# dgkuester/iqwaveform

Measured on NVIDIA B200. Metric: complex IQ GS/s for persistence_spectrum, higher is better.
Workload: dtype f32

## Files before the change

### include/iqw_b200.h

```cpp
#ifndef IQW_B200_H
#define IQW_B200_H

#include <stddef.h>
#include <stdint.h>

#ifdef __cplusplus
extern "C" {
#endif

#define IQW_ABI_VERSION 8

typedef enum iqw_status {
    IQW_OK = 0,
    IQW_ERR_INVALID = -1,
    IQW_ERR_UNSUPPORTED = -2,
    IQW_ERR_CUDA = -3,
    IQW_ERR_WORKSPACE = -4
} iqw_status;

typedef enum iqw_stft_mode {
    IQW_STFT_COMPLEX = 0,
    IQW_STFT_POWER = 1,
    IQW_STFT_DB = 2
} iqw_stft_mode;
// ... 72 lines not shown
                       const float* d_window, int32_t nfft, int64_t hop, int64_t n_frames,
                       int32_t bin_lo, int32_t bin_hi, void* d_out, int64_t out_channel_stride,
                       void* stream);


int iqw_edge_counts_f32(const float* d_a, int64_t n_rows, int64_t n_cols, const double* d_edges,
                        int32_t n_edges, int32_t side_right, int64_t* d_counts, void* stream);

size_t iqw_bracket_collect_workspace_bytes(int64_t n_rows, int64_t n_cols);
int iqw_bracket_collect_f32(const float* d_p, int64_t n_rows, int64_t n_cols, int32_t n_sel,
                            const uint32_t* d_lo, const uint32_t* d_hi, int32_t* d_below,
                            void* d_workspace, size_t workspace_bytes, void* stream);
int iqw_candidate_count_f32(const void* d_workspace, int64_t n_rows, int64_t n_cols, int32_t n_sel,
                            const uint32_t* d_lo, const uint32_t* d_hi, int32_t level,
                            int32_t* d_counts, void* stream);
int iqw_radix_count_f32(const float* d_p, int64_t n_rows, int64_t n_cols, int32_t n_sel,
                        const uint32_t* d_lo, const uint32_t* d_hi, int32_t level,
                        int32_t* d_counts, int32_t* d_below, void* stream);
int iqw_radix_descend(const int32_t* d_counts, int32_t n_sel, int64_t n_cols, int32_t level,
                      int64_t* d_rank, uint32_t* d_prefix, uint32_t* d_lo, uint32_t* d_hi,
                      void* stream);
int iqw_order_stats_finish_f32(const uint32_t* d_keys, int32_t n_sel, const int64_t* sel_rank,
                               int64_t n_rows_total, int64_t n_cols, const iqw_stat* stats,
                               int32_t n_stats, int32_t to_dB, float eps, float* d_out, void* stream);

int iqw_debug_set_stft_scratch_cap(size_t bytes);

int iqw_debug_set_sample_min_rows(int64_t rows);

int iqw_debug_set_stft_variant(int variant);

int iqw_debug_set_sample_margin(double sigmas, int extra_ranks);

int iqw_debug_time_stats_counters(const void* d_workspace, int64_t n_cols, uint32_t* host_out16);

int iqw_profile_enable(int level);
int iqw_profile_reset(void);
int iqw_profile_report(char* buf, size_t capacity);

#ifdef __cplusplus
}
#endif
#endif
```

### iqwaveform_b200/_lib.py

```python
from __future__ import annotations

import ctypes
import os

import torch

_HERE = os.path.dirname(os.path.abspath(__file__))
LIB_PATH = os.environ.get('IQW_B200_LIB') or os.path.join(_HERE, 'libiqw_b200.so')

ABI_VERSION = 8

IQW_OK = 0
IQW_ERR_INVALID = -1
IQW_ERR_UNSUPPORTED = -2
IQW_ERR_CUDA = -3
IQW_ERR_WORKSPACE = -4

STFT_COMPLEX, STFT_POWER, STFT_DB = 0, 1, 2
STAT_QUANTILE, STAT_MEAN, STAT_MAX, STAT_MIN, STAT_MEDIAN, STAT_ORDER = 0, 1, 2, 3, 4, 5
EW_POWTODB, EW_DBTOPOW, EW_ENVTOPOW, EW_ENVTODB = 0, 1, 2, 3

MAX_RANKS_PER_CALL = 8


# ... 17 lines not shown
                                    _i32, _i32, _vp, _i64, _vp, _sz, _vp]),
    'iqw_stft_bluestein_c64': (ctypes.c_int, [_vp, _i64, _i64, _i64, _vp, _vp, _vp, _i32, _i32, _i64, _i64, _i32, _f32,
                                              _i32, _i32, _vp, _i64, _vp]),
    'iqw_bluestein_pre_c64': (ctypes.c_int, [_vp, _i64, _vp, _i32, _i32, _i64, _vp, _vp]),
    'iqw_bluestein_mul_c64': (ctypes.c_int, [_vp, _vp, _i32, _i64, _vp]),
    'iqw_bluestein_post_c64': (ctypes.c_int, [_vp, _vp, _i32, _i64, _i32, _f32, _i32, _i32, _vp, _vp]),
    'iqw_stft_reduce_workspace_bytes': (_sz, [_i32]),
    'iqw_stft_reduce_c64': (ctypes.c_int, [_vp, _i64, _i64, _i64, _vp, _i32, _i64, _i64, _i32, _f32, _i32, _i32,
                                           ctypes.POINTER(iqw_stat), _i32, _vp, _vp, _sz, _vp]),
    'iqw_time_stats_workspace_bytes': (_sz, [_i64, _i64, _i64, _i32]),
    'iqw_time_stats_f32': (ctypes.c_int, [_vp, _i64, _i64, _i64, _i64, ctypes.POINTER(iqw_stat),
                                          _i32, _i32, _f32, _vp, _vp, _sz, _vp]),
    'iqw_bin_power_workspace_bytes': (_sz, [_i64, _i64, _i64]),
    'iqw_bin_power_c64': (ctypes.c_int, [_vp, _i64, _i64, _i64, _i64, _vp, _vp, _vp, _vp, _sz, _vp]),
    'iqw_envtopow_transposed_c64': (ctypes.c_int, [_vp, _i64, _i64, _i64, _i64, _vp, _vp]),
    'iqw_elementwise_f32': (ctypes.c_int, [_i32, _vp, _vp, _i64, _i32, _f32, _vp]),
    'iqw_elementwise_c64': (ctypes.c_int, [_i32, _vp, _vp, _i64, _f32, _vp]),
    'iqw_transpose_c64': (ctypes.c_int, [_vp, _i64, _i64, _i64, _vp, _vp]),
    'iqw_istft_c64': (ctypes.c_int, [_vp, _i64, _i64, _i64, _i32, _i64, _i32, _i32, _i32, _vp, _f32, _vp, _i64, _vp]),
    'iqw_ifft_c64': (ctypes.c_int, [_vp, _i64, _i32, _vp, _vp]),
    'iqw_ola_filter_c64': (ctypes.c_int, [_vp, _i64, _i64, _i64, _vp, _i32, _i64, _i64, _i32, _i32, _vp, _i64, _vp]),
    'iqw_edge_counts_f32': (ctypes.c_int, [_vp, _i64, _i64, _vp, _i32, _i32, _vp, _vp]),
    'iqw_bracket_collect_workspace_bytes': (_sz, [_i64, _i64]),
    'iqw_bracket_collect_f32': (ctypes.c_int, [_vp, _i64, _i64, _i32, _vp, _vp, _vp, _vp, _sz, _vp]),
    'iqw_candidate_count_f32': (ctypes.c_int, [_vp, _i64, _i64, _i32, _vp, _vp, _i32, _vp, _vp]),
    'iqw_radix_count_f32': (ctypes.c_int, [_vp, _i64, _i64, _i32, _vp, _vp, _i32, _vp, _vp, _vp]),
    'iqw_radix_descend': (ctypes.c_int, [_vp, _i32, _i64, _i32, _vp, _vp, _vp, _vp, _vp]),
    'iqw_order_stats_finish_f32': (ctypes.c_int, [_vp, _i32, ctypes.POINTER(_i64), _i64, _i64,
                                                  ctypes.POINTER(iqw_stat), _i32, _i32, _f32, _vp, _vp]),
    'iqw_debug_set_stft_scratch_cap': (ctypes.c_int, [_sz]),
    'iqw_debug_set_stft_variant': (ctypes.c_int, [ctypes.c_int]),
    'iqw_debug_set_sample_min_rows': (ctypes.c_int, [_i64]),
    'iqw_debug_set_sample_margin': (ctypes.c_int, [ctypes.c_double, ctypes.c_int]),
    'iqw_debug_time_stats_counters': (ctypes.c_int, [_vp, _i64, ctypes.POINTER(ctypes.c_uint32)]),
    'iqw_profile_enable': (ctypes.c_int, [ctypes.c_int]),
    'iqw_profile_reset': (ctypes.c_int, []),
    'iqw_profile_report': (ctypes.c_int, [ctypes.c_char_p, _sz]),
}


def _load() -> ctypes.CDLL:
    if not os.path.exists(LIB_PATH):
        raise ImportError(
            f'{LIB_PATH} is missing: build it with `python -c "import __graft_entry__ as g; '
            f'g.build()"` or `make -C iqwaveform_b200/csrc`.  iqwaveform_b200 has no CPU fallback.'
        )
    lib = ctypes.CDLL(LIB_PATH)
    for name, (restype, argtypes) in SIGNATURES.items():
        try:
            fn = getattr(lib, name)
        except AttributeError as exc:
            raise ImportError(f'{LIB_PATH} does not export {name}') from exc
        fn.restype = restype
        fn.argtypes = argtypes
    got = lib.iqw_abi_version()
    if got != ABI_VERSION:
        raise ImportError(f'{LIB_PATH}: ABI version {got}, python layer expects {ABI_VERSION}')
    return lib


lib = _load()


class IQWError(RuntimeError):
    pass

# ... 26 lines not shown
```

### iqwaveform_b200/csrc/iqw_stats.cu

```cuda
#include <cmath>
#include <atomic>
#include <cooperative_groups.h>
#include "iqw_common.cuh"

namespace iqw {

constexpr int kMaxRanks = 8;
constexpr int kMaxStats = 32;
constexpr int kNB0 = 256;
constexpr int kNSub = 32;
constexpr int kCap = 2048;
constexpr int kRefineLevels = 7;
constexpr int kBX = 128;
#ifndef IQW_UNROLL
#define IQW_UNROLL 8
#endif
constexpr int kUnroll = IQW_UNROLL;
constexpr long long kSampleMinRows = 16384;
constexpr int kSampleRows = 8192;
#ifndef IQW_SAMPLE_COLS
#define IQW_SAMPLE_COLS 2
#endif
constexpr int kSampleCols = IQW_SAMPLE_COLS;
constexpr int kMaxGroups = 8;
constexpr int kSelBins = 2048;
constexpr int kSubBins = 256;
#ifndef IQW_SEL_BUF
#define IQW_SEL_BUF 2048
#endif
#ifndef IQW_SEL_THREADS
#define IQW_SEL_THREADS 512
#endif
// ... 361 lines not shown
        }
        cum = next;
    }
    iv_store(L, w, col);
}

__device__ void scan_refine_body(long long col, long long cols, const RankPlan& rp, const Work& w) {
    if (col >= cols) return;
    IvList O, L;
    iv_load(O, w, col);
    bool any = false;
    for (uint32_t v = 0; v < O.n; ++v) any |= O.status[v] == IV_REFINE;
    if (!any) return;
    L.n = 0;
    for (uint32_t v = 0; v < O.n; ++v) {
        if (O.status[v] != IV_REFINE) {
            const uint32_t i = L.n++;
            L.klo[i] = O.klo[v]; L.khi[i] = O.khi[v]; L.shift[i] = O.shift[v]; L.below[i] = O.below[v];
            L.status[i] = O.status[v]; L.first[i] = O.first[v]; L.nr[i] = O.nr[v]; L.cnt[i] = O.cnt[v];
            continue;
        }
        atomicSub(w.pending, 1u);
        uint32_t cum = O.below[v], i = O.first[v];
        split_by_subbuckets(L, O, v, w.hist1 + (col * kMaxRanks + v) * kNSub, rp, i, cum, w, col);
    }
    iv_store(L, w, col);
}

__global__ void scan_refine_kernel(long long cols, RankPlan rp, Work w) {
    if (*w.pending == 0) return;
    scan_refine_body((long long)blockIdx.x * blockDim.x + threadIdx.x, cols, rp, w);
}

__global__ void scan_brackets_kernel(long long cols, long long rows, RankPlan rp, int n_groups,
                                     Work w) {
    const long long col = (long long)blockIdx.x * blockDim.x + threadIdx.x;
    if (col >= cols) return;
    IvList L;
    L.n = 0;
    uint32_t i = 0;
    const uint32_t nrk = (uint32_t)rp.n_ranks;
    const uint32_t ovf = w.t_ovf[col];
    bool first_live = true;
    for (int g = 0; g < n_groups && i < nrk; ++g) {
        const uint32_t lo = w.bk_lo[col * kMaxGroups + g], hi = w.bk_hi[col * kMaxGroups + g];
        if (lo > hi) continue;
        const uint32_t below = w.t_below[col * kMaxGroups + g];
        unsigned long long next_lo = 0x100000000ull;
        uint32_t next_below = (uint32_t)rows;
        for (int h = g + 1; h < n_groups; ++h) {
            const uint32_t l2 = w.bk_lo[col * kMaxGroups + h];
            if (l2 <= w.bk_hi[col * kMaxGroups + h]) { next_lo = l2; next_below = w.t_below[col * kMaxGroups + h]; break; }
        }
        if (first_live && rp.rank[i] < below) {
            const uint32_t first = i;
            while (i < nrk && rp.rank[i] < below) ++i;
            atomicAdd(w.pending + 2, i - first);
            iv_append(L, w, col, 0u, (unsigned long long)lo, 0u, below, first, i - first, false, 0u);
        }
        first_live = false;
        if (i < nrk && rp.rank[i] < next_below) {
            const uint32_t first = i;
            while (i < nrk && rp.rank[i] < next_below) ++i;
            const uint32_t region = next_below - below;
            if (ovf) {
                atomicAdd(w.pending + 3, 1u);
                iv_append(L, w, col, lo, next_lo - lo, below, region, first, i - first, false, 0u);
            } else {
                const uint32_t v = L.n++;
                L.klo[v] = lo; L.khi[v] = hi; L.below[v] = below; L.cnt[v] = region;
// ... 91 lines not shown
refine_kernel(const float* __restrict__ p, long long cols, RowMap rm, long long rows_per_split,
              Work w) {
    if (*w.pending == 0) return;
    extern __shared__ uint16_t hist[];
    refine_body<M>(blockIdx.x, blockIdx.y, gridDim.x, p, cols, rm, rows_per_split, w, hist);
}

#include "bracket_visit.inc"

template <bool RAW, int M>
__device__ __forceinline__ void bracket_visit_generic(uint32_t v, float (&nge)[M], float (&nin)[M],
                                                      uint32_t& slot, const uint32_t (&lo)[M],
                                                      const uint32_t (&hi)[M], uint32_t base) {
    bool inside = false;
#pragma unroll
    for (int g = 0; g < M; ++g) {
        const bool ge = RAW ? (int32_t)v >= (int32_t)lo[g] : v >= lo[g];
        const bool in = ge && (RAW ? (int32_t)v <= (int32_t)hi[g] : v <= hi[g]);
        nge[g] += ge ? 1.f : 0.f;
        nin[g] += in ? 1.f : 0.f;
        inside |= in;
    }
    if (inside) {
        asm volatile("st.shared.u32 [%0], %1;" :: "r"(base + 4 * slot), "r"(v) : "memory");
        slot += 1;
    }
}

constexpr int kLine = 32;
constexpr int kStage = kLine + kUnroll;
constexpr int kStagePitch = kStage + 1;

template <int M, int NAMED , bool RAW>
__device__ __forceinline__ void bracket_pass_body(const float* __restrict__ p, long long cols, long long col,
                                                  bool live_col, long long i0, long long i1, float eps,
                                                  const BracketPlan& bp, const Work& w, uint32_t* stage) {
    uint32_t lo[M], hi[M];
    float n_ge[M], n_in[M];
#pragma unroll
    for (int g = 0; g < M; ++g) {
        lo[g] = (live_col ? w.bk_lo[col * kMaxGroups + g] : 0xFFFFFFFFu) ^ (RAW ? 0x80000000u : 0u);
        hi[g] = (live_col ? w.bk_hi[col * kMaxGroups + g] : 0u) ^ (RAW ? 0x80000000u : 0u);
        n_ge[g] = 0.f; n_in[g] = 0.f;
    }
    const uint32_t cap = bp.cap_sum;
    const int lane = threadIdx.x & 31;
    uint32_t* my_stage = stage + threadIdx.x * kStagePitch;
    const uint32_t* warp_stage = stage + (threadIdx.x - lane) * kStagePitch;
    const uint32_t stage_addr = (uint32_t)__cvta_generic_to_shared(my_stage);
    uint32_t slot = 0;
    uint32_t n_lines = 0;
    uint32_t* warp_list = w.lists + ((long long)blockIdx.y * cols + (long long)blockIdx.x * kBX +
                                     (threadIdx.x - lane)) * (long long)cap;
    Named<(NAMED & 1) != 0, (NAMED & 2) != 0, (NAMED & 4) != 0> named;

    auto drain = [&](bool ready) {
        unsigned m = __ballot_sync(0xFFFFFFFFu, ready);
        __syncwarp();
        while (m) {
            const int src = __ffs(m) - 1;
            m &= m - 1;
            const uint32_t start = __shfl_sync(0xFFFFFFFFu, n_lines, src) * kLine;
            if (start + kLine <= cap)
                warp_list[(uint32_t)src * cap + start + lane] = warp_stage[src * kStagePitch + lane];
        }
        __syncwarp();
        if (ready) {
            const uint32_t left = slot - kLine;
            uint32_t t[kUnroll];
#pragma unroll
            for (int j = 0; j < kUnroll; ++j) t[j] = my_stage[kLine + j];
#pragma unroll
            for (int j = 0; j < kUnroll; ++j)
                if ((uint32_t)j < left) my_stage[j] = t[j];
            slot -= kLine;
            ++n_lines;
        }
    };
    auto visit = [&](float f) {
        const uint32_t bits = __float_as_uint(f);
        if (NAMED) named.add(f, float_to_key(f), eps);
        const uint32_t v = RAW ? bits : float_to_key(f);
        if constexpr (M <= 4) bracket_visit<RAW>(v, n_ge, n_in, slot, lo, hi, stage_addr);
        else bracket_visit_generic<RAW, M>(v, n_ge, n_in, slot, lo, hi, stage_addr);
    };
// ... 113 lines not shown
        for (int u = 0; u < kBpUnroll; ++u) visit(f[u]);
        drain(kChunk);
    };
    if (i + kBpUnroll <= i1) load_block(fa);
#pragma unroll 1
    while (i + kBpUnroll <= i1) {
        if (i + 2 * kBpUnroll <= i1) load_block(fb);
        visit_block(fa);
        i += kBpUnroll;
        if (i + kBpUnroll > i1) break;
        if (i + 2 * kBpUnroll <= i1) load_block(fa);
        visit_block(fb);
        i += kBpUnroll;
    }
#pragma unroll 1
    for (; i < i1; ++i, src += cols) {
        visit(__ldcs(src));
    }
    drain(kChunk);
    const uint32_t n_list = p4 >> 2;
    drain(1u);
    if (!live_col) return;

#pragma unroll
    for (int g = 0; g < M; ++g)
        if (g < bp.n_groups && wd[g] != 0u && nlt[g]) atomicAdd(w.t_below + col * kMaxGroups + g, nlt[g]);
    w.s_cnt[(long long)blockIdx.y * cols + col] = min(n_list, cap);
    if (n_list > cap) atomicOr(w.t_ovf + col, 1u);
    named.flush(w, col);
}

template <int M, int NAMED>
__global__ void __launch_bounds__(kBX)
bracket_pass_kernel(const float* __restrict__ p, long long cols, long long rows,
                    long long rows_per_split, float eps, BracketPlan bp, Work w) {
    static_assert(kRing <= kStagePitch, "the staging area serves both bodies");
    __shared__ __align__(128) uint32_t stage[kBX * kStagePitch];
    long long col = (long long)blockIdx.x * kBX + threadIdx.x;
    const bool live_col = col < cols;
    if (!live_col) col = cols - 1;
    const long long i0 = (long long)blockIdx.y * rows_per_split;
    const long long i1 = min(rows, i0 + rows_per_split);
    if (w.pending[8] == 0) {
        if constexpr (M <= 4) bracket_pass_body_diff<M, NAMED>(p, cols, col, live_col, i0, i1, eps, bp, w, stage);
        else bracket_pass_body<M, NAMED, true>(p, cols, col, live_col, i0, i1, eps, bp, w, stage);
    } else {
        bracket_pass_body<M, NAMED, false>(p, cols, col, live_col, i0, i1, eps, bp, w, stage);
    }
}

template <int M>
__device__ __forceinline__ void collect_body(unsigned bx, unsigned by, unsigned gdx, const float* __restrict__ p,
                                             long long cols, RowMap rm, long long rows_per_split, const Work& w) {
    const long long col_tiles = (cols + kBX - 1) / kBX;
    const long long i0 = (long long)by * rows_per_split;
    const long long i1 = min(rm.n, i0 + rows_per_split);
    for (long long tile = bx; tile < col_tiles; tile += gdx) {
        const long long col = tile * kBX + threadIdx.x;
        int active = 0;
        IvRegs<M> iv;
        iv.load(w, col, col < cols, IV_COLLECT, active);
        if (!__syncthreads_or(active)) continue;
        if (!active) continue;
        auto visit = [&](float f) {
            const uint32_t k = float_to_key(f);
            uint32_t kl, kh, sh;
            const int v = iv.find(k, kl, kh, sh);
            if (v >= 0 && k <= kh && sh < 32u) {
                const long long x = col * kMaxRanks + v;
                const uint32_t pos = atomicAdd(w.cursor + x, 1u);
                if (pos < (uint32_t)kCap) w.cand[x * kCap + pos] = k;
            }
        };
        IQW_STREAM(rm.step != 1, p, cols, col, rm, i0, i1, visit);
    }
}

template <int M>
__global__ void __launch_bounds__(kBX)
collect_kernel(const float* __restrict__ p, long long cols, RowMap rm, long long rows_per_split,
// ... 222 lines not shown
    }
    __syncthreads();

    if (t < kSampleCols && c0 + t < cols) {
        const long long col = c0 + t;
        int last = -1;
        uint32_t last_hi = 0u;
        bool not_raw = false;
        for (int g = 0; g < kMaxGroups; ++g) {
            uint32_t lo = 0xFFFFFFFFu, hi = 0u;
            if (g < bp.n_groups) {
                lo = bp.s_lo[g] < 0 ? 0u : s_elo[t][bp.s_lo[g]];
                hi = bp.s_hi[g] < 0 ? 0xFFFFFFFFu : s_ehi[t][bp.s_hi[g]];
                if (hi < lo) hi = lo;
                if (last >= 0 && lo <= last_hi) {
                    if (hi > last_hi) { last_hi = hi; w.bk_hi[col * kMaxGroups + last] = hi; }
                    lo = 0xFFFFFFFFu; hi = 0u;
                } else {
                    last = g; last_hi = hi;
                }
            }
            w.bk_lo[col * kMaxGroups + g] = lo;
            w.bk_hi[col * kMaxGroups + g] = hi;
            not_raw |= lo <= hi && ((lo != 0u && lo <= 0x80000000u) || hi < 0x80000000u);
        }
        if (not_raw) atomicOr(w.pending + 8, 1u);
    }
}

enum SelMode : uint32_t { SEL_IDLE = 0, SEL_HIST = 1, SEL_COLLECT = 2 };

template <int M>
__global__ void __launch_bounds__(kSelThreads, IQW_SEL_MINBLOCKS)
select_kernel(long long cols, int splits, RankPlan rp, BracketPlan bp, Work w) {
    extern __shared__ uint32_t smem_u32[];
    uint32_t* hist = smem_u32;
    uint32_t* buf = hist + M * kSelBins;
    uint32_t* cnts = buf + M * kSelBuf;
    __shared__ uint32_t s_a[M], s_b[M], s_sh[M], s_below[M], s_first[M], s_nr[M], s_iv[M];
    __shared__ uint32_t s_bf[M], s_bl[M], s_cb[M], s_n[M], s_mode[M];
    __shared__ uint32_t s_region[M], s_gap_hi[M], s_out_first[M], s_out_nr[M], s_out_below[M], s_out_cnt[M], s_keep[M];
    __shared__ int s_any, s_rebuild;
    __shared__ uint4 s_tbl[M + 1];
    __shared__ uint32_t s_thr[M + 1];

    const long long col = blockIdx.x;
    const int t = threadIdx.x, lane = t & 31, warp = t >> 5;
    constexpr int NW = kSelThreads / 32;
    if (t < M) { s_mode[t] = SEL_IDLE; s_iv[t] = 0xFFFFFFFFu; s_n[t] = 0; s_a[t] = 0xFFFFFFFFu; s_b[t] = 0; s_sh[t] = 0;
                 s_out_nr[t] = 0; s_keep[t] = 1; }
    if (t == 0) { s_any = 0; s_rebuild = 0; }
    __syncthreads();
    if (t < kMaxRanks && (uint32_t)t < w.n_iv[col]) {
        const long long x = col * kMaxRanks + t;
        const uint32_t status = w.iv_status[x], g = w.iv_shift[x];
        const uint32_t klo = w.iv_klo[x], khi = w.iv_khi[x], below = w.iv_below[x], first = w.iv_first[x], nr = w.iv_nr[x];
        if (status == IV_SELECT && g < (uint32_t)M) {
            s_iv[g] = (uint32_t)t;
            s_a[g] = klo; s_b[g] = khi;
            s_sh[g] = sel_shift(khi - klo, kSelBins);
            s_below[g] = below; s_first[g] = first; s_nr[g] = nr;
            s_region[g] = w.t_cnt[col * kMaxGroups + g]; s_gap_hi[g] = w.t_gap_hi[col * kMaxGroups + g];
            s_mode[g] = SEL_HIST;
            s_any = 1;
        }
    }
    for (int i = t; i < splits; i += kSelThreads) cnts[i] = w.s_cnt[(long long)i * cols + col];
    __syncthreads();
    if (!s_any) return;

    const uint32_t cap_sum = bp.cap_sum;
    const bool raw = w.pending[8] == 0;
    const uint32_t key_or = raw ? 0x80000000u : 0u, key_and = raw ? 0x7FFFFFFFu : 0u;
    auto key_of = [&](uint32_t v) {
        return v ^ ((((uint32_t)((int32_t)v >> 31)) & key_and) | key_or);
    };
    auto sweep = [&](bool keep, auto&& visit) {
        const size_t stride = (size_t)cols * cap_sum;
        const uint32_t* src = w.lists + (size_t)col * cap_sum + (size_t)warp * stride + 4 * lane;
// ... 355 lines not shown
            if (lo < 0 || hi < lo || hi >= rows)
                return fail(IQW_ERR_INVALID, "statistic %d: ranks (%lld, %lld) outside [0, %lld)", i,
                            (long long)lo, (long long)hi, (long long)rows);
            ranks[nr++] = lo;
            ranks[nr++] = hi;
        }
    }
    for (int i = 1; i < nr; ++i)
        for (int j = i; j > 0 && ranks[j] < ranks[j - 1]; --j) {
            int64_t tmp = ranks[j]; ranks[j] = ranks[j - 1]; ranks[j - 1] = tmp;
        }
    int nu = 0;
    for (int i = 0; i < nr; ++i)
        if (nu == 0 || ranks[i] != ranks[nu - 1]) ranks[nu++] = ranks[i];
    if (nu > kMaxRanks)
        return fail(IQW_ERR_UNSUPPORTED,
                    "%d distinct order statistics requested; at most %d per call (split the request)",
                    nu, kMaxRanks);
    rp->n_ranks = nu;
    for (int i = 0; i < nu; ++i) rp->rank[i] = (unsigned)ranks[i];
    for (int i = 0; i < n_stats; ++i) {
        const iqw_stat& s = stats[i];
        if (s.kind != IQW_STAT_QUANTILE && s.kind != IQW_STAT_MEDIAN && s.kind != IQW_STAT_ORDER) continue;
        const int64_t lo = s.kind == IQW_STAT_MEDIAN ? (rows - 1) / 2 : s.rank_lo;
        const int64_t hi = s.kind == IQW_STAT_MEDIAN ? rows / 2 : s.kind == IQW_STAT_ORDER ? s.rank_lo : s.rank_hi;
        for (int k = 0; k < nu; ++k) {
            if (ranks[k] == lo) st->ia[i] = k;
            if (ranks[k] == hi) st->ib[i] = k;
        }
    }
    return IQW_OK;
}

static std::atomic<double> g_margin_sigmas{5.0};
static std::atomic<int> g_margin_extra{2};
static std::atomic<long long> g_sample_min_rows{kSampleMinRows};
constexpr long long kSampleRowsMin = 2048;
static std::atomic<long long> g_sample_share{8};

struct LongPlan {
    long long splits, rows_per_split;
    RowMap sample;
    BracketPlan bp;
};

static void plan_long_shape(int64_t rows, int64_t cols, LongPlan* lp) {
    const long long col_tiles = (cols + kBX - 1) / kBX;
    long long splits = kBracketCtas / col_tiles;
    if (splits < 1) splits = 1;
    if (splits > kMaxSplits) splits = kMaxSplits;
    long long rps = (rows + splits - 1) / splits;
    if (rps < kMinRowsPerSplit) rps = kMinRowsPerSplit;
    lp->rows_per_split = rps;
    lp->splits = (rows + rps - 1) / rps;
    long long want = rows / g_sample_share.load();
    if (want < kSampleRowsMin) want = kSampleRowsMin;
    if (want > kSampleRows) want = kSampleRows;
    long long step = (rows + want - 1) / want;
    if (step < 2) step = 2;
    lp->sample = RowMap{rows / step, step, 0x9E3779B9u};
}

static long long max_group_width(long long srows) {
    return 2 * ((long long)std::ceil(6.0 * std::sqrt((double)srows * 0.25)) + 2) + 3;
}

// ... 68 lines not shown
    g->grid = dim3((unsigned)col_tiles, (unsigned)splits);
    g->rows_per_split = rps;
    return IQW_OK;
}

template <int M>
static void launch_refine_levels(const Grid& g, cudaStream_t s, const float* p, long long cols,
                                 RowMap rm, const RankPlan& rp, const Work& w, unsigned cblocks,
                                 unsigned cthreads, const char* tag) {
    static const char* const names[2][kRefineLevels] = {
        {"stats_refine_1", "stats_refine_2", "stats_refine_3", "stats_refine_4", "stats_refine_5",
         "stats_refine_6", "stats_refine_7"},
        {"sample_refine_1", "sample_refine_2", "sample_refine_3", "sample_refine_4",
         "sample_refine_5", "sample_refine_6", "sample_refine_7"}};
    const int which = tag[1] == 'a' ? 1 : 0;
    const size_t smem = sizeof(uint16_t) * M * kNSub * kBX;
    cudaFuncSetAttribute(refine_kernel<M>, cudaFuncAttributeMaxDynamicSharedMemorySize, (int)smem);
    for (int level = 0; level < kRefineLevels; ++level) {
        { IQW_PROFILE_FINE(names[which][level], s);
          refine_kernel<M><<<g.grid, kBX, smem, s>>>(p, cols, rm, g.rows_per_split, w); }
        { IQW_PROFILE_FINE(which ? "sample_scan" : "stats_scan", s);
          scan_refine_kernel<<<cblocks, cthreads, 0, s>>>(cols, rp, w); }
    }
}

template <int M>
static void launch_collect(const Grid& g, cudaStream_t s, const float* p, long long cols, RowMap rm,
                           const Work& w, const char* name) {
    IQW_PROFILE_FINE(name, s);
    collect_kernel<M><<<g.grid, kBX, 0, s>>>(p, cols, rm, g.rows_per_split, w);
}

template <int M>
static void launch_bracket_pass(cudaStream_t s, const float* p, long long cols, long long rows,
                                const LongPlan& lp, bool want_minmax, bool want_sum, bool to_dB, float eps,
                                const Work& w) {
    const dim3 grid((unsigned)((cols + kBX - 1) / kBX), (unsigned)lp.splits);
    IQW_PROFILE("stats_bracket_pass", s);
#define IQW_BP(N) bracket_pass_kernel<M, N><<<grid, kBX, 0, s>>>(p, cols, rows, lp.rows_per_split, eps, lp.bp, w)
    const int named = (want_minmax ? 1 : 0) | (want_sum ? 2 : 0) | (want_sum && to_dB ? 4 : 0);
    switch (named) {
        case 0: IQW_BP(0); break;
        case 1: IQW_BP(1); break;
        case 2: IQW_BP(2); break;
        case 3: IQW_BP(3); break;
        case 6: IQW_BP(6); break;
        default: IQW_BP(7); break;
    }
#undef IQW_BP
}

template <int M>
static int launch_tail(cudaStream_t s, const TailArgs& a, int sms) {
    constexpr size_t smem_refine = sizeof(uint16_t) * M * kNSub * kBX, smem_keys = sizeof(uint32_t) * kCap;
    constexpr size_t smem = smem_refine > smem_keys ? smem_refine : smem_keys;
    static std::atomic<int> blocks_per_sm[64];
    int dev = 0;
    IQW_CUDA_OK(cudaGetDevice(&dev));
    if (dev < 0 || dev >= 64) return IQW_ERR_UNSUPPORTED;
    int bps = blocks_per_sm[dev].load();
    if (bps == 0) {
        int coop = 0;
        IQW_CUDA_OK(cudaDeviceGetAttribute(&coop, cudaDevAttrCooperativeLaunch, dev));
        IQW_CUDA_OK(cudaFuncSetAttribute(tail_kernel<M>, cudaFuncAttributeMaxDynamicSharedMemorySize, (int)smem));
        IQW_CUDA_OK(cudaOccupancyMaxActiveBlocksPerMultiprocessor(&bps, tail_kernel<M>, kBX, smem));
        if (!coop || bps < 1) bps = -1;
        else if (bps > 8) bps = 8;
        blocks_per_sm[dev].store(bps);
    }
    if (bps < 0) return IQW_ERR_UNSUPPORTED;
    TailArgs args = a;
    void* params[] = {&args};
    if (cudaLaunchCooperativeKernel((const void*)tail_kernel<M>, dim3((unsigned)(sms * bps)), dim3(kBX), params, smem, s) !=
        cudaSuccess) {
        (void)cudaGetLastError();
        return IQW_ERR_UNSUPPORTED;
    }
    return IQW_OK;
}

template <int M>
static int launch_select(cudaStream_t s, long long cols, const RankPlan& rp, const LongPlan& lp, const Work& w) {
    const size_t smem = sizeof(uint32_t) * ((size_t)M * (kSelBins + kSelBuf) + (size_t)lp.splits);
    IQW_CUDA_OK(cudaFuncSetAttribute(select_kernel<M>, cudaFuncAttributeMaxDynamicSharedMemorySize, (int)smem));
    IQW_PROFILE("stats_select", s);
    select_kernel<M><<<(unsigned)cols, kSelThreads, smem, s>>>(cols, (int)lp.splits, rp, lp.bp, w);
    return IQW_OK;
}

#define IQW_DISPATCH_G(m, CALL)                  \
    do {                                         \
        if ((m) <= 1) { constexpr int M = 1; CALL; }        \
        else if ((m) <= 2) { constexpr int M = 2; CALL; }   \
        else if ((m) <= 4) { constexpr int M = 4; CALL; }   \
        else { constexpr int M = 8; CALL; }                 \
    } while (0)

#define IQW_DISPATCH_M(m, CALL)                  \
    do {                                         \
        if ((m) <= 2) { constexpr int M = 2; CALL; }        \
        else if ((m) <= 4) { constexpr int M = 4; CALL; }   \
        else { constexpr int M = 8; CALL; }                 \
    } while (0)

static int run_exact(const float* p, long long cols, RowMap rm, const RankPlan& rp, bool named,
                     bool want_sum, bool to_dB, float eps, const Work& w, int sms, cudaStream_t s,
                     bool sample) {
    const long long col_tiles = (cols + kBX - 1) / kBX;
    Grid g;
    if (int rc = plan_grid(rm.n, col_tiles, sms, &g)) return rc;
    const unsigned cthreads = 128, cblocks = (unsigned)((cols + cthreads - 1) / cthreads);

    long long stride = rm.n / 2048;
    if (stride < 1) stride = 1;
    long long rsplits = (rm.n + stride - 1) / stride / 64;
    if (rsplits < 1) rsplits = 1;
    if (rsplits > 64) rsplits = 64;
    IQW_PROFILE_TRAIN(sample ? "sample_exact" : "stats_exact", s, rp.n_ranks > 0 ? 3 + 2 * kRefineLevels + 2 : 2);
    { IQW_PROFILE_FINE(sample ? "sample_range" : "stats_range", s);
// ... 7 lines not shown
        cudaFuncSetAttribute(l0_kernel<A, B, C>, cudaFuncAttributeMaxDynamicSharedMemorySize, (int)l0_smem); \
        l0_kernel<A, B, C><<<g.grid, kBX, l0_smem, s>>>(p, cols, rm, g.rows_per_split, eps, w);       \
    } while (0)
        if (!named) IQW_L0(false, false, false);
        else if (want_sum && to_dB) IQW_L0(true, true, true);
        else if (want_sum) IQW_L0(true, true, false);
        else IQW_L0(true, false, false);
#undef IQW_L0
    }
    if (rp.n_ranks > 0) {
        { IQW_PROFILE_FINE(sample ? "sample_scan" : "stats_scan", s);
          scan0_kernel<<<cblocks, cthreads, 0, s>>>(cols, rp, w); }
        IQW_DISPATCH_M(rp.n_ranks, launch_refine_levels<M>(g, s, p, cols, rm, rp, w, cblocks, cthreads,
                                                           sample ? "sample" : "stats"));
        IQW_DISPATCH_M(rp.n_ranks, launch_collect<M>(g, s, p, cols, rm, w,
                                                     sample ? "sample_collect" : "stats_collect"));
        { IQW_PROFILE_FINE(sample ? "sample_resolve" : "stats_resolve", s);
          resolve_kernel<<<(unsigned)cols, kResolveThreads, 0, s>>>(cols, rp, w); }
    }
    IQW_CUDA_OK(cudaGetLastError());
    return IQW_OK;
}

static int reset_work(const Work& w, cudaStream_t s) {
    IQW_CUDA_OK(cudaMemsetAsync(w.range_hi, 0, w.zero_bytes, s));
    IQW_CUDA_OK(cudaMemsetAsync(reinterpret_cast<char*>(w.range_hi) + w.zero_bytes, 0xFF, w.ff_bytes, s));
    return IQW_OK;
}

}

using namespace iqw;

extern "C" int iqw_debug_set_sample_margin(double sigmas, int extra) {
    g_margin_sigmas = sigmas;
    g_margin_extra = extra;
    return IQW_OK;
}

extern "C" int iqw_debug_set_sample_min_rows(int64_t rows) {
    if (rows < 0) { g_sample_share.store(-rows); return IQW_OK; }
    if (rows == 0) g_sample_share.store(8);
    g_sample_min_rows.store(rows < 1 ? kSampleMinRows : rows);
    return IQW_OK;
}

extern "C" int iqw_debug_time_stats_counters(const void* d_workspace, int64_t n_cols, uint32_t* host_out16) {
    if (!d_workspace || !host_out16 || n_cols < 1) return fail(IQW_ERR_INVALID, "bad argument");
    Work w{};
    carve_work(const_cast<void*>(d_workspace), n_cols, 0, 0, &w);
    IQW_CUDA_OK(cudaMemcpy(host_out16, w.pending, 16 * sizeof(uint32_t), cudaMemcpyDeviceToHost));
    return IQW_OK;
}

extern "C" size_t iqw_time_stats_workspace_bytes(int64_t n_channels, int64_t n_rows, int64_t n_cols,
                                                 int32_t n_stats) {
    (void)n_channels;
    if (n_cols <= 0) return 256;
    if (n_rows < g_sample_min_rows.load() || n_stats < 1) return carve_work(nullptr, n_cols, 0, 0, nullptr);
    LongPlan lp{};
    plan_long_shape(n_rows, n_cols, &lp);
    const int groups = n_stats < kMaxGroups ? n_stats : kMaxGroups;
    return carve_work(nullptr, n_cols, lp.splits, cap_budget(lp, groups), nullptr);
}

extern "C" int iqw_time_stats_f32(const float* d_p, int64_t n_channels, int64_t n_rows,
// ... 9 lines not shown
    if (n_rows >= 0xFFFFFFFFll) return fail(IQW_ERR_UNSUPPORTED, "n_rows >= 2^32");
    if (((uintptr_t)d_workspace & 255) != 0) return fail(IQW_ERR_INVALID, "workspace not 256-byte aligned");

    RankPlan rp{};
    StatPlan st{};
    bool want_sum = false, want_minmax = false;
    if (int rc = build_plans(stats, n_stats, n_rows, &rp, &st, &want_sum)) return rc;
    for (int i = 0; i < n_stats; ++i)
        want_minmax |= stats[i].kind == IQW_STAT_MAX || stats[i].kind == IQW_STAT_MIN;
    if (n_cols >= (1ll << 27)) return fail(IQW_ERR_UNSUPPORTED, "n_cols >= 2^27");

    LongPlan lp{};
    const bool sampled = n_rows >= g_sample_min_rows.load() && rp.n_ranks > 0 &&
                         build_long_plan(rp, n_rows, n_cols, n_stats, &lp);
    Work w{};
    const size_t need = sampled ? carve_work(d_workspace, n_cols, lp.splits, lp.bp.cap_sum, &w)
                                : carve_work(d_workspace, n_cols, 0, 0, &w);
    if (workspace_bytes < need)
        return fail(IQW_ERR_WORKSPACE, "workspace %zu bytes < required %zu", workspace_bytes, need);

    cudaStream_t s = static_cast<cudaStream_t>(stream);
    int sms = 0;
    if (int rc = device_sm_count(&sms)) return rc;
    const long long col_tiles = (n_cols + kBX - 1) / kBX;
    const unsigned cthreads = 128, cblocks = (unsigned)((n_cols + cthreads - 1) / cthreads);
    RowMap full{n_rows, 1, 0u};
    if (sampled)
        IQW_CUDA_OK(cudaFuncSetAttribute(sample_brackets_kernel, cudaFuncAttributeMaxDynamicSharedMemorySize,
                                         (int)kSampleSmem));

    for (int64_t c = 0; c < n_channels; ++c) {
        const float* p = d_p + c * p_channel_stride;
        float* out = d_out + c * (int64_t)n_stats * n_cols;
        { IQW_PROFILE_FINE("stats_init", s); if (int rc = reset_work(w, s)) return rc; }

        if (!sampled) {
            if (int rc = run_exact(p, n_cols, full, rp, true, want_sum, to_dB != 0, eps, w, sms, s, false))
                return rc;
        } else {
            { IQW_PROFILE("stats_sample", s);
              sample_brackets_kernel<<<(unsigned)((n_cols + kSampleCols - 1) / kSampleCols), kSampleThreads,
                                       kSampleSmem, s>>>(p, n_cols, lp.sample, lp.bp, w); }
            IQW_DISPATCH_G(lp.bp.n_groups, launch_bracket_pass<M>(s, p, n_cols, n_rows, lp, want_minmax, want_sum, to_dB != 0, eps, w));
            { IQW_PROFILE("stats_scan", s);
              scan_brackets_kernel<<<cblocks, cthreads, 0, s>>>(n_cols, n_rows, rp, lp.bp.n_groups, w); }
            IQW_DISPATCH_G(lp.bp.n_groups, if (int rc = launch_select<M>(s, n_cols, rp, lp, w)) return rc);
            Grid g;
            {
                const long long slots = col_tiles < 4 ? col_tiles : 4;
                long long splits = (32ll * sms + slots - 1) / slots;
                long long rps = (n_rows + splits - 1) / splits;
                if (rps < 4 * kUnroll) rps = 4 * kUnroll;
                if (rps > 65535) rps = 65535;
                splits = (n_rows + rps - 1) / rps;
                if (splits > 65535) return fail(IQW_ERR_UNSUPPORTED, "too many rows for the split grid");
                g.grid = dim3((unsigned)slots, (unsigned)splits);
                g.rows_per_split = rps;
            }
            TailArgs ta{p, n_rows, n_cols, full, g.grid.x, g.grid.y, g.rows_per_split, rp, st, to_dB, eps, w, out};
            int rc_tail = IQW_OK;
            { IQW_PROFILE("stats_tail", s);
              IQW_DISPATCH_M(rp.n_ranks, rc_tail = launch_tail<M>(s, ta, sms)); }
            if (rc_tail == IQW_ERR_UNSUPPORTED) {
                IQW_PROFILE_TRAIN("stats_tail_train", s, 2 * kRefineLevels + 3);
                IQW_DISPATCH_M(rp.n_ranks, launch_refine_levels<M>(g, s, p, n_cols, full, rp, w, cblocks, cthreads, "stats"));
                IQW_DISPATCH_M(rp.n_ranks, launch_collect<M>(g, s, p, n_cols, full, w, "stats_collect"));
                { IQW_PROFILE_FINE("stats_resolve", s);
                  resolve_kernel<<<(unsigned)n_cols, kResolveThreads, 0, s>>>(n_cols, rp, w); }
                { IQW_PROFILE_FINE("stats_finalize", s);
                  finalize_kernel<<<cblocks, cthreads, 0, s>>>(n_rows, n_cols, st, to_dB, eps, w, out); }
            } else if (rc_tail != IQW_OK) {
                return rc_tail;
            }
        }
        if (!sampled) {
            IQW_PROFILE("stats_finalize", s);
            finalize_kernel<<<cblocks, cthreads, 0, s>>>(n_rows, n_cols, st, to_dB, eps, w, out);
        }
        IQW_CUDA_OK(cudaGetLastError());
// ... 4 lines not shown
```

### iqwaveform_b200/csrc/iqw_stft2p.cu

```cuda
#include <mutex>
#include <map>
#include <utility>
#include <atomic>
#include "iqw_stft.cuh"

#ifndef IQW_P2_SLOTS12
#define IQW_P2_SLOTS12 6
#endif
#ifndef IQW_P2_SLOTS11
#define IQW_P2_SLOTS11 12
#endif

namespace iqw {

template <int LOG2N, bool STAGED = true>
struct P2Cfg {
    static constexpr int N = 1 << LOG2N;
    static constexpr int RA = LOG2N >= 11 ? 64 : 32;
    static constexpr int RB = N / RA;
    static constexpr int E = RA;
    static constexpr int TPF = N / E;
    static constexpr int NB = E / RB;
    static constexpr int SLOTS = LOG2N == 12 ? (STAGED ? IQW_P2_SLOTS12 : 4) : LOG2N == 11 ? (STAGED ? IQW_P2_SLOTS11 : 8) : 8;
    static constexpr int THREADS = SLOTS * TPF;
    static constexpr int MIN_BLOCKS = LOG2N == 10 ? 2 : 1;
    static constexpr int ROW = RA + 2;
    static constexpr int BUF = RB * ROW;
    static constexpr int NA8 = RB / 8;
    static constexpr int TW_ROWS = (NA8 - 1) + 7;
    static constexpr int TW = TW_ROWS * RA;
    static constexpr size_t SMEM = sizeof(float2) * ((size_t)TW + (size_t)SLOTS * BUF);
    static_assert(RA >= RB && RA * RB == N && TPF == RB && TPF % 32 == 0, "geometry");
    static_assert((ROW * sizeof(float2)) % 16 == 0 && ((ROW * sizeof(float2)) / 16) % 2 == 1, "row padding");
};

__device__ __forceinline__ float2 ldg_stream(const float2* p) {
    float2 v;
    asm volatile("ld.global.nc.L1::no_allocate.v2.f32 {%0, %1}, [%2];" : "=f"(v.x), "=f"(v.y) : "l"(p));
    return v;
}

__device__ __forceinline__ uint32_t smem_u32(const void* p) { return (uint32_t)__cvta_generic_to_shared(p); }
__device__ __forceinline__ void mbar_init(uint64_t* bar, int count) {
    asm volatile("mbarrier.init.shared::cta.b64 [%0], %1;" ::"r"(smem_u32(bar)), "r"(count) : "memory");
}
__device__ __forceinline__ void mbar_expect_tx(uint64_t* bar, uint32_t bytes) {
    asm volatile("mbarrier.arrive.expect_tx.shared::cta.b64 _, [%0], %1;" ::"r"(smem_u32(bar)), "r"(bytes) : "memory");
}
__device__ __forceinline__ void mbar_wait(uint64_t* bar, uint32_t parity) {
    asm volatile(
        "{\n\t.reg .pred p;\n\t"
        "WAIT_%=:\n\t"
        "mbarrier.try_wait.parity.shared::cta.b64 p, [%0], %1;\n\t"
        "@p bra DONE_%=;\n\t"
        "bra WAIT_%=;\n\t"
        "DONE_%=:\n\t}" ::"r"(smem_u32(bar)), "r"(parity) : "memory");
}
__device__ __forceinline__ void bulk_load(void* dst_smem, const void* src_gmem, uint32_t bytes, uint64_t* bar) {
    asm volatile("cp.async.bulk.shared::cluster.global.mbarrier::complete_tx::bytes [%0], [%1], %2, [%3];" ::"r"(
                     smem_u32(dst_smem)),
                 "l"(src_gmem), "r"(bytes), "r"(smem_u32(bar))
                 : "memory");
}
__device__ __forceinline__ void fence_proxy_async() { asm volatile("fence.proxy.async.shared::cta;" ::: "memory"); }

template <int LOG2N, int MODE, bool FULLBAND, bool STAGED>
__global__ void __launch_bounds__(P2Cfg<LOG2N, STAGED>::THREADS, P2Cfg<LOG2N, STAGED>::MIN_BLOCKS)
stft2p_kernel(const StftArgs a) {
    using C = P2Cfg<LOG2N, STAGED>;
    constexpr int RA = C::RA, RB = C::RB, E = C::E, TPF = C::TPF, NB = C::NB, ROW = C::ROW;

    extern __shared__ __align__(16) unsigned char smem_raw[];
    float2* tw = reinterpret_cast<float2*>(smem_raw);
    __shared__ __align__(8) uint64_t full_bar[C::SLOTS];
    for (int i = threadIdx.x; i < C::TW; i += C::THREADS) tw[i] = a.twiddle[i];
    if constexpr (STAGED) {
        if (threadIdx.x < C::SLOTS) mbar_init(&full_bar[threadIdx.x], 1);
        asm volatile("fence.mbarrier_init.release.cluster;" ::: "memory");
        fence_proxy_async();
    }
    __syncthreads();

    const int slot = threadIdx.x / TPF;
    const int ltid = threadIdx.x % TPF;
    float2* buf = tw + C::TW + (size_t)slot * C::BUF;
    constexpr uint32_t kFrameBytes = (uint32_t)(C::N * sizeof(float2));
    static_assert(!STAGED || C::BUF >= C::N, "the exchange buffer doubles as the staging buffer");

    auto slot_sync = [&]() {
        if constexpr (TPF == 32) __syncwarp();
        else asm volatile("bar.sync %0, %1;" ::"r"(slot + 1), "n"(TPF) : "memory");
    };

    const long long total = (long long)a.n_channels * a.n_frames;
    const long long n_slots = (long long)gridDim.x * C::SLOTS;
    const long long per = (total + n_slots - 1) / n_slots;
    const long long sg = (long long)blockIdx.x * C::SLOTS + slot;
    long long f = sg * per;
    const long long f_end = f + per < total ? f + per : total;
    if (f >= f_end) return;
// ... 486 lines not shown
```

Measured before the change: 146.6.

## Overlap stats bracket pass with scan/select via column chunks on side stream

Splits the sampled time-stats path into column chunks: bracket-pass kernels for each chunk run on the main stream and record events, while scan and select for finished chunks run on a high-priority side stream. The aim is to hide the scan/select tail behind the remaining bracket passes instead of running them back to back. In exchange it adds extra launches, per-device cached streams and events, and more concurrent kernels competing for SMs. Debug knobs for stage masks and chunk count, plus a launch-bound macro, are also added.

```diff
diff --git a/include/iqw_b200.h b/include/iqw_b200.h
--- a/include/iqw_b200.h
+++ b/include/iqw_b200.h
@@ -128,6 +128,10 @@
 
 int iqw_debug_set_sample_margin(double sigmas, int extra_ranks);
 
+int iqw_debug_set_stats_stages(int mask);
+
+int iqw_debug_set_stats_col_chunks(int chunks);
+
 int iqw_debug_time_stats_counters(const void* d_workspace, int64_t n_cols, uint32_t* host_out16);
 
 int iqw_profile_enable(int level);
diff --git a/iqwaveform_b200/_lib.py b/iqwaveform_b200/_lib.py
--- a/iqwaveform_b200/_lib.py
+++ b/iqwaveform_b200/_lib.py
@@ -73,6 +73,8 @@
     'iqw_debug_set_stft_variant': (ctypes.c_int, [ctypes.c_int]),
     'iqw_debug_set_sample_min_rows': (ctypes.c_int, [_i64]),
     'iqw_debug_set_sample_margin': (ctypes.c_int, [ctypes.c_double, ctypes.c_int]),
+    'iqw_debug_set_stats_stages': (ctypes.c_int, [ctypes.c_int]),
+    'iqw_debug_set_stats_col_chunks': (ctypes.c_int, [ctypes.c_int]),
     'iqw_debug_time_stats_counters': (ctypes.c_int, [_vp, _i64, ctypes.POINTER(ctypes.c_uint32)]),
     'iqw_profile_enable': (ctypes.c_int, [ctypes.c_int]),
     'iqw_profile_reset': (ctypes.c_int, []),
diff --git a/iqwaveform_b200/csrc/iqw_stats.cu b/iqwaveform_b200/csrc/iqw_stats.cu
--- a/iqwaveform_b200/csrc/iqw_stats.cu
+++ b/iqwaveform_b200/csrc/iqw_stats.cu
@@ -1,3 +1,4 @@
+#include <algorithm>
 #include <cmath>
 #include <atomic>
 #include <cooperative_groups.h>
@@ -425,10 +426,10 @@
     scan_refine_body((long long)blockIdx.x * blockDim.x + threadIdx.x, cols, rp, w);
 }
 
-__global__ void scan_brackets_kernel(long long cols, long long rows, RankPlan rp, int n_groups,
-                                     Work w) {
-    const long long col = (long long)blockIdx.x * blockDim.x + threadIdx.x;
-    if (col >= cols) return;
+__global__ void scan_brackets_kernel(long long cols, long long c0, long long c1, long long rows, RankPlan rp,
+                                     int n_groups, Work w) {
+    const long long col = c0 + (long long)blockIdx.x * blockDim.x + threadIdx.x;
+    if (col >= c1) return;
     IvList L;
     L.n = 0;
     uint32_t i = 0;
@@ -586,8 +587,8 @@
 constexpr int kStagePitch = kStage + 1;
 
 template <int M, int NAMED , bool RAW>
-__device__ __forceinline__ void bracket_pass_body(const float* __restrict__ p, long long cols, long long col,
-                                                  bool live_col, long long i0, long long i1, float eps,
+__device__ __forceinline__ void bracket_pass_body(const float* __restrict__ p, long long cols, long long col0,
+                                                  long long col, bool live_col, long long i0, long long i1, float eps,
                                                   const BracketPlan& bp, const Work& w, uint32_t* stage) {
     uint32_t lo[M], hi[M];
     float n_ge[M], n_in[M];
@@ -604,7 +605,7 @@
     const uint32_t stage_addr = (uint32_t)__cvta_generic_to_shared(my_stage);
     uint32_t slot = 0;
     uint32_t n_lines = 0;
-    uint32_t* warp_list = w.lists + ((long long)blockIdx.y * cols + (long long)blockIdx.x * kBX +
+    uint32_t* warp_list = w.lists + ((long long)blockIdx.y * cols + col0 + (long long)blockIdx.x * kBX +
                                      (threadIdx.x - lane)) * (long long)cap;
     Named<(NAMED & 1) != 0, (NAMED & 2) != 0, (NAMED & 4) != 0> named;
 
@@ -784,20 +785,20 @@
 
 template <int M, int NAMED>
 __global__ void __launch_bounds__(kBX)
-bracket_pass_kernel(const float* __restrict__ p, long long cols, long long rows,
+bracket_pass_kernel(const float* __restrict__ p, long long cols, long long col0, long long rows,
                     long long rows_per_split, float eps, BracketPlan bp, Work w) {
     static_assert(kRing <= kStagePitch, "the staging area serves both bodies");
     __shared__ __align__(128) uint32_t stage[kBX * kStagePitch];
-    long long col = (long long)blockIdx.x * kBX + threadIdx.x;
+    long long col = col0 + (long long)blockIdx.x * kBX + threadIdx.x;
     const bool live_col = col < cols;
     if (!live_col) col = cols - 1;
     const long long i0 = (long long)blockIdx.y * rows_per_split;
     const long long i1 = min(rows, i0 + rows_per_split);
     if (w.pending[8] == 0) {
         if constexpr (M <= 4) bracket_pass_body_diff<M, NAMED>(p, cols, col, live_col, i0, i1, eps, bp, w, stage);
-        else bracket_pass_body<M, NAMED, true>(p, cols, col, live_col, i0, i1, eps, bp, w, stage);
+        else bracket_pass_body<M, NAMED, true>(p, cols, col0, col, live_col, i0, i1, eps, bp, w, stage);
     } else {
-        bracket_pass_body<M, NAMED, false>(p, cols, col, live_col, i0, i1, eps, bp, w, stage);
+        bracket_pass_body<M, NAMED, false>(p, cols, col0, col, live_col, i0, i1, eps, bp, w, stage);
     }
 }
 
@@ -1086,7 +1087,7 @@
 
 template <int M>
 __global__ void __launch_bounds__(kSelThreads, IQW_SEL_MINBLOCKS)
-select_kernel(long long cols, int splits, RankPlan rp, BracketPlan bp, Work w) {
+select_kernel(long long cols, long long col0, int splits, RankPlan rp, BracketPlan bp, Work w) {
     extern __shared__ uint32_t smem_u32[];
     uint32_t* hist = smem_u32;
     uint32_t* buf = hist + M * kSelBins;
@@ -1098,7 +1099,7 @@
     __shared__ uint4 s_tbl[M + 1];
     __shared__ uint32_t s_thr[M + 1];
 
-    const long long col = blockIdx.x;
+    const long long col = col0 + blockIdx.x;
     const int t = threadIdx.x, lane = t & 31, warp = t >> 5;
     constexpr int NW = kSelThreads / 32;
     if (t < M) { s_mode[t] = SEL_IDLE; s_iv[t] = 0xFFFFFFFFu; s_n[t] = 0; s_a[t] = 0xFFFFFFFFu; s_b[t] = 0; s_sh[t] = 0;
@@ -1520,6 +1521,32 @@
     return IQW_OK;
 }
 
+static std::atomic<int> g_stats_stages{7};
+constexpr int kMaxColChunks = 16;
+#ifndef IQW_COL_CHUNKS
+#define IQW_COL_CHUNKS 4
+#endif
+static std::atomic<int> g_stats_col_chunks{IQW_COL_CHUNKS};
+
+struct SideStream {
+    cudaStream_t side = nullptr;
+    cudaEvent_t ev[kMaxColChunks + 1] = {};
+};
+static int side_stream(SideStream** out) {
+    thread_local SideStream cache[64];
+    int dev = 0;
+    IQW_CUDA_OK(cudaGetDevice(&dev));
+    if (dev < 0 || dev >= 64) return fail(IQW_ERR_UNSUPPORTED, "device index %d", dev);
+    SideStream& ss = cache[dev];
+    if (!ss.side) {
+        int lo = 0, hi = 0;
+        IQW_CUDA_OK(cudaDeviceGetStreamPriorityRange(&lo, &hi));
+        for (auto& e : ss.ev) IQW_CUDA_OK(cudaEventCreateWithFlags(&e, cudaEventDisableTiming));
+        IQW_CUDA_OK(cudaStreamCreateWithPriority(&ss.side, cudaStreamNonBlocking, hi));
+    }
+    *out = &ss;
+    return IQW_OK;
+}
 static std::atomic<double> g_margin_sigmas{5.0};
 static std::atomic<int> g_margin_extra{2};
 static std::atomic<long long> g_sample_min_rows{kSampleMinRows};
@@ -1654,12 +1681,12 @@
 }
 
 template <int M>
-static void launch_bracket_pass(cudaStream_t s, const float* p, long long cols, long long rows,
-                                const LongPlan& lp, bool want_minmax, bool want_sum, bool to_dB, float eps,
-                                const Work& w) {
-    const dim3 grid((unsigned)((cols + kBX - 1) / kBX), (unsigned)lp.splits);
-    IQW_PROFILE("stats_bracket_pass", s);
-#define IQW_BP(N) bracket_pass_kernel<M, N><<<grid, kBX, 0, s>>>(p, cols, rows, lp.rows_per_split, eps, lp.bp, w)
+static void launch_bracket_pass(cudaStream_t s, const float* p, long long cols, long long tile0, long long tile1,
+                                long long rows, const LongPlan& lp, bool want_minmax, bool want_sum, bool to_dB,
+                                float eps, const Work& w) {
+    const dim3 grid((unsigned)(tile1 - tile0), (unsigned)lp.splits);
+    const long long col0 = tile0 * kBX;
+#define IQW_BP(N) bracket_pass_kernel<M, N><<<grid, kBX, 0, s>>>(p, cols, col0, rows, lp.rows_per_split, eps, lp.bp, w)
     const int named = (want_minmax ? 1 : 0) | (want_sum ? 2 : 0) | (want_sum && to_dB ? 4 : 0);
     switch (named) {
         case 0: IQW_BP(0); break;
@@ -1702,11 +1729,11 @@
 }
 
 template <int M>
-static int launch_select(cudaStream_t s, long long cols, const RankPlan& rp, const LongPlan& lp, const Work& w) {
+static int launch_select(cudaStream_t s, long long cols, long long c0, long long c1, const RankPlan& rp,
+                         const LongPlan& lp, const Work& w) {
     const size_t smem = sizeof(uint32_t) * ((size_t)M * (kSelBins + kSelBuf) + (size_t)lp.splits);
     IQW_CUDA_OK(cudaFuncSetAttribute(select_kernel<M>, cudaFuncAttributeMaxDynamicSharedMemorySize, (int)smem));
-    IQW_PROFILE("stats_select", s);
-    select_kernel<M><<<(unsigned)cols, kSelThreads, smem, s>>>(cols, (int)lp.splits, rp, lp.bp, w);
+    select_kernel<M><<<(unsigned)(c1 - c0), kSelThreads, smem, s>>>(cols, c0, (int)lp.splits, rp, lp.bp, w);
     return IQW_OK;
 }
 
@@ -1780,6 +1807,18 @@
 
 using namespace iqw;
 
+extern "C" int iqw_debug_set_stats_col_chunks(int chunks) {
+    if (chunks < 0 || chunks > kMaxColChunks) return fail(IQW_ERR_INVALID, "chunks %d outside 0..%d", chunks, kMaxColChunks);
+    g_stats_col_chunks.store(chunks ? chunks : IQW_COL_CHUNKS);
+    return IQW_OK;
+}
+
+extern "C" int iqw_debug_set_stats_stages(int mask) {
+    if (mask < 0 || mask > 7) return fail(IQW_ERR_INVALID, "stage mask %d outside 0..7", mask);
+    g_stats_stages.store(mask ? mask : 7);
+    return IQW_OK;
+}
+
 extern "C" int iqw_debug_set_sample_margin(double sigmas, int extra) {
     g_margin_sigmas = sigmas;
     g_margin_extra = extra;
@@ -1855,19 +1894,58 @@
     for (int64_t c = 0; c < n_channels; ++c) {
         const float* p = d_p + c * p_channel_stride;
         float* out = d_out + c * (int64_t)n_stats * n_cols;
-        { IQW_PROFILE_FINE("stats_init", s); if (int rc = reset_work(w, s)) return rc; }
+        const int stages = sampled ? g_stats_stages.load() : 7;
+        if (stages & 1) { IQW_PROFILE_FINE("stats_init", s); if (int rc = reset_work(w, s)) return rc; }
 
         if (!sampled) {
             if (int rc = run_exact(p, n_cols, full, rp, true, want_sum, to_dB != 0, eps, w, sms, s, false))
                 return rc;
         } else {
-            { IQW_PROFILE("stats_sample", s);
-              sample_brackets_kernel<<<(unsigned)((n_cols + kSampleCols - 1) / kSampleCols), kSampleThreads,
-                                       kSampleSmem, s>>>(p, n_cols, lp.sample, lp.bp, w); }
-            IQW_DISPATCH_G(lp.bp.n_groups, launch_bracket_pass<M>(s, p, n_cols, n_rows, lp, want_minmax, want_sum, to_dB != 0, eps, w));
-            { IQW_PROFILE("stats_scan", s);
-              scan_brackets_kernel<<<cblocks, cthreads, 0, s>>>(n_cols, n_rows, rp, lp.bp.n_groups, w); }
-            IQW_DISPATCH_G(lp.bp.n_groups, if (int rc = launch_select<M>(s, n_cols, rp, lp, w)) return rc);
+            if (stages & 1) {
+                IQW_PROFILE("stats_sample", s);
+                sample_brackets_kernel<<<(unsigned)((n_cols + kSampleCols - 1) / kSampleCols), kSampleThreads,
+                                         kSampleSmem, s>>>(p, n_cols, lp.sample, lp.bp, w);
+            }
+            long long chunks = stages == 7 ? g_stats_col_chunks.load() : 1;
+            if (chunks > col_tiles) chunks = col_tiles;
+            if (chunks <= 1) {
+                if (stages & 2) {
+                    IQW_PROFILE("stats_bracket_pass", s);
+                    IQW_DISPATCH_G(lp.bp.n_groups, launch_bracket_pass<M>(s, p, n_cols, 0, col_tiles, n_rows, lp, want_minmax,
+                                                                          want_sum, to_dB != 0, eps, w));
+                }
+                if (!(stages & 4)) { IQW_CUDA_OK(cudaGetLastError()); continue; }
+                { IQW_PROFILE("stats_scan", s);
+                  scan_brackets_kernel<<<cblocks, cthreads, 0, s>>>(n_cols, 0, n_cols, n_rows, rp, lp.bp.n_groups, w); }
+                IQW_PROFILE("stats_select", s);
+                IQW_DISPATCH_G(lp.bp.n_groups, if (int rc = launch_select<M>(s, n_cols, 0, n_cols, rp, lp, w)) return rc);
+            } else {
+                SideStream* ss = nullptr;
+                if (int rc = side_stream(&ss)) return rc;
+                {
+                    IQW_PROFILE("stats_bracket_pass", s);
+                    for (long long k = 0; k < chunks; ++k) {
+                        const long long t0 = col_tiles * k / chunks, t1 = col_tiles * (k + 1) / chunks;
+                        IQW_DISPATCH_G(lp.bp.n_groups, launch_bracket_pass<M>(s, p, n_cols, t0, t1, n_rows, lp, want_minmax,
+                                                                              want_sum, to_dB != 0, eps, w));
+                        IQW_CUDA_OK(cudaEventRecord(ss->ev[k], s));
+                    }
+                }
+                IQW_CUDA_OK(cudaStreamWaitEvent(ss->side, ss->ev[0], 0));
+                {
+                    IQW_PROFILE("stats_select", ss->side);
+                    for (long long k = 0; k < chunks; ++k) {
+                        const long long c0 = col_tiles * k / chunks * kBX;
+                        const long long c1 = std::min<long long>(n_cols, col_tiles * (k + 1) / chunks * kBX);
+                        if (k) IQW_CUDA_OK(cudaStreamWaitEvent(ss->side, ss->ev[k], 0));
+                        scan_brackets_kernel<<<(unsigned)((c1 - c0 + cthreads - 1) / cthreads), cthreads, 0, ss->side>>>(
+                            n_cols, c0, c1, n_rows, rp, lp.bp.n_groups, w);
+                        IQW_DISPATCH_G(lp.bp.n_groups, if (int rc = launch_select<M>(ss->side, n_cols, c0, c1, rp, lp, w)) return rc);
+                    }
+                }
+                IQW_CUDA_OK(cudaEventRecord(ss->ev[kMaxColChunks], ss->side));
+                IQW_CUDA_OK(cudaStreamWaitEvent(s, ss->ev[kMaxColChunks], 0));
+            }
             Grid g;
             {
                 const long long slots = col_tiles < 4 ? col_tiles : 4;
diff --git a/iqwaveform_b200/csrc/iqw_stft2p.cu b/iqwaveform_b200/csrc/iqw_stft2p.cu
--- a/iqwaveform_b200/csrc/iqw_stft2p.cu
+++ b/iqwaveform_b200/csrc/iqw_stft2p.cu
@@ -9,6 +9,9 @@
 #endif
 #ifndef IQW_P2_SLOTS11
 #define IQW_P2_SLOTS11 12
+#endif
+#ifndef IQW_P2_BOUND12
+#define IQW_P2_BOUND12 0
 #endif
 
 namespace iqw {
@@ -23,6 +26,7 @@
     static constexpr int NB = E / RB;
     static constexpr int SLOTS = LOG2N == 12 ? (STAGED ? IQW_P2_SLOTS12 : 4) : LOG2N == 11 ? (STAGED ? IQW_P2_SLOTS11 : 8) : 8;
     static constexpr int THREADS = SLOTS * TPF;
+    static constexpr int BOUND_THREADS = LOG2N == 12 && STAGED && IQW_P2_BOUND12 > 0 ? IQW_P2_BOUND12 : THREADS;
     static constexpr int MIN_BLOCKS = LOG2N == 10 ? 2 : 1;
     static constexpr int ROW = RA + 2;
     static constexpr int BUF = RB * ROW;
@@ -65,7 +69,7 @@
 __device__ __forceinline__ void fence_proxy_async() { asm volatile("fence.proxy.async.shared::cta;" ::: "memory"); }
 
 template <int LOG2N, int MODE, bool FULLBAND, bool STAGED>
-__global__ void __launch_bounds__(P2Cfg<LOG2N, STAGED>::THREADS, P2Cfg<LOG2N, STAGED>::MIN_BLOCKS)
+__global__ void __launch_bounds__(P2Cfg<LOG2N, STAGED>::BOUND_THREADS, P2Cfg<LOG2N, STAGED>::MIN_BLOCKS)
 stft2p_kernel(const StftArgs a) {
     using C = P2Cfg<LOG2N, STAGED>;
     constexpr int RA = C::RA, RB = C::RB, E = C::E, TPF = C::TPF, NB = C::NB, ROW = C::ROW;
diff --git a/sweep_tmp.py b/sweep_tmp.py
--- /dev/null
+++ b/sweep_tmp.py
@@ -0,0 +1,23 @@
+import sys, os, json
+sys.path.insert(0, os.getcwd())
+import torch, bench
+import iqwaveform_b200 as iqw
+from iqwaveform_b200 import _lib
+dev = torch.device('cuda', 0)
+x = bench.device_capture(torch, 1_000_000_000, 1, dev)
+kw = dict(fs=100e6, window='hann', resolution=100e6 / 4096, fractional_overlap=0.5, statistics=[0.1, 0.5, 0.9, 0.999], dB=True)
+res = {}
+refs = {}
+for rep in range(3):
+    for k in (1, 2, 4, 8, 16):
+        _lib.check(_lib.lib.iqw_debug_set_stats_col_chunks(k))
+        o = iqw.persistence_spectrum(x, **kw); torch.cuda.synchronize()
+        refs.setdefault(k, o)
+        assert torch.equal(o, refs[1]), k
+        e0, e1 = torch.cuda.Event(enable_timing=True), torch.cuda.Event(enable_timing=True)
+        e0.record()
+        for _ in range(10):
+            iqw.persistence_spectrum(x, **kw)
+        e1.record(); torch.cuda.synchronize()
+        res.setdefault(k, []).append(round(e0.elapsed_time(e1) / 10, 4))
+print('sweep', json.dumps(res))
```

After: 141.7 (median of 6 runs). -3.4%, worse.
